# rounak-meyur/revs-admm

Measured on NVIDIA B200. Metric: home_hours_scheduled_per_sec, higher is better.
Workload: dtype f64

## Files before the change

include/revs_admm.h:

```cpp
#ifndef REVS_ADMM_H
#define REVS_ADMM_H

#include <stdint.h>

#ifdef __cplusplus
extern "C" {
#endif

#define REVS_OK 0
#define REVS_ERR_ARG 1
#define REVS_ERR_CUDA 2
#define REVS_ERR_INFEASIBLE 3
#define REVS_ERR_NOCONV 4

#define REVS_REL_VOLTAGE 0
#define REVS_REL_FLOW 1
#define REVS_REL_DROP 2

typedef struct revs_solver revs_solver;

typedef struct revs_stats {
    int64_t kernel_launches;
    int64_t gemm_launches;
    int64_t gemm_full_launches;
// ... 3 lines not shown
    int32_t max_working_set;
    double primal_residual;
    double dual_residual;
    double qp_flops;
    float gemm_ms;
    float gemm_full_ms;
    float home_ms;
    float dual_ms;
    float qp_ms;
    float qp_big_ms;
    float total_ms;
    float qp_warp_ms;
    float qp_init_ms;
    int64_t qp_columns;
    int64_t qp_warp_rounds;
} revs_stats;

const char* revs_last_error(void);
int revs_version(void);
int revs_device_count(int* count);

int revs_create(revs_solver** out, int device, int n_feeders, const int64_t* feeder_off, int T);
int revs_destroy(revs_solver* s);

int revs_set_sensitivity(revs_solver* s, int feeder, const double* R_res);

int revs_set_feeder_tree(revs_solver* s, int feeder, int n_nodes, const int32_t* parent,
                         const double* r, const int32_t* res_node);

int revs_set_feeder_trees(revs_solver* s, const int64_t* node_off, const int32_t* parent,
// ... 61 lines not shown
```

revs-admm_b200/_cabi.py:

```python
import ctypes as C
import os

import numpy as np

HERE = os.path.dirname(os.path.abspath(__file__))
LIB_PATH = os.environ.get("REVS_LIB") or os.path.join(HERE, "librevs_admm.so")

REVS_REL_VOLTAGE, REVS_REL_FLOW, REVS_REL_DROP = 0, 1, 2


class RevsError(RuntimeError):
    def __init__(self, code, msg):
        super().__init__(f"revs_admm error {code}: {msg}")
        self.code = code


class Stats(C.Structure):
    _fields_ = [("kernel_launches", C.c_int64), ("gemm_launches", C.c_int64), ("gemm_full_launches", C.c_int64),
                ("qp_outer_iterations", C.c_int64), ("qp_newton_iterations", C.c_int64),
                ("admm_iterations", C.c_int32), ("max_working_set", C.c_int32),
                ("primal_residual", C.c_double), ("dual_residual", C.c_double), ("qp_flops", C.c_double),
                ("gemm_ms", C.c_float), ("gemm_full_ms", C.c_float), ("home_ms", C.c_float), ("dual_ms", C.c_float),
                ("qp_ms", C.c_float), ("qp_big_ms", C.c_float), ("total_ms", C.c_float),
                ("qp_warp_ms", C.c_float), ("qp_init_ms", C.c_float), ("qp_columns", C.c_int64),
                ("qp_warp_rounds", C.c_int64)]

    def as_dict(self):
        return {k: getattr(self, k) for k, _ in self._fields_}


_P = C.c_void_p
_D = C.POINTER(C.c_double)
SIGNATURES = {
    "revs_last_error": ([], C.c_char_p),
    "revs_version": ([], C.c_int),
    "revs_device_count": ([C.POINTER(C.c_int)], C.c_int),
    "revs_create": ([C.POINTER(_P), C.c_int, C.c_int, C.POINTER(C.c_int64), C.c_int], C.c_int),
    "revs_destroy": ([_P], C.c_int),
    "revs_set_sensitivity": ([_P, C.c_int, _D], C.c_int),
    "revs_set_feeder_tree": ([_P, C.c_int, C.c_int, C.POINTER(C.c_int32), _D, C.POINTER(C.c_int32)], C.c_int),
    "revs_set_feeder_trees": ([_P, C.POINTER(C.c_int64), C.POINTER(C.c_int32), _D, C.POINTER(C.c_int32)], C.c_int),
    "revs_set_homes": ([_P, _D, C.POINTER(C.c_uint8), _D, _D, _D, C.POINTER(C.c_int32),
                        C.POINTER(C.c_int32)], C.c_int),
# ... 320 lines not shown
```

revs-admm_b200/csrc/kernels.cuh:

```cuda
#pragma once
#include <vector>

#include "common.cuh"

namespace revs {

struct HomeParams {
    const double* load;
    const double* p_est;
    const double* p_sch;
    const int* iter;
    const double* gamma;
    const double* cost;
    const uint8_t* has_ev;
    const double* rating;
    const int* start;
    const int* end;
    const int* n_min;
    const int* n_max;
    double* p_sch_new;
    double* p_ev;
    double* dsum;
    int first;
    int* infeasible;
// ... 115 lines not shown
struct ClassGateParams {
    const int* order_count;
    unsigned long long cond[kQpClasses];
    int first_gated;
};
cudaError_t launch_class_gate(const ClassGateParams& P, cudaStream_t stream);
cudaError_t qp_warp_prepare();
cudaError_t screen_prepare();
cudaError_t screen_tc5_prepare();

cudaError_t launch_utility_qp(const QpParams& P, int grid, int cls, cudaStream_t stream);
int qp_warp_max_n();
cudaError_t launch_qp_init(const QpParams& P, int max_warp_n, cudaStream_t stream);
int qp_warp_ctas_per_sm();
int qp_warp_m_max_default();
cudaError_t launch_utility_qp_warp(const QpParams& P, int nj, int ctas_per_sm, cudaStream_t stream);
cudaError_t launch_utility_qp_fast(const QpParams& P, cudaStream_t stream);
cudaError_t launch_order_columns(const QpParams& P, int mode, int* order, int* order_count, cudaStream_t stream);

struct TreeParams {
    const int64_t* zoff;
    const int* perm;
    const int* iperm;
    const double* c;
    const double* d;
    const double* e;
    const int* nodeA;
    const double* wA;
    const int* permB;
    const int* cnt;
    int* left;
// ... 99 lines not shown
```

revs-admm_b200/csrc/revs_capi.cu:

```cuda
#include <chrono>
#include <cstdarg>
#include <cstdio>
#include <cstring>
#include <algorithm>
#include <cstdlib>
#include <cmath>
#include <mutex>
#include <string>
#include <vector>

#include "../../include/revs_admm.h"
#include "kernels.cuh"

using namespace revs;

namespace {

thread_local std::string g_err;

int fail(int code, const char* fmt, ...) {
    char buf[512];
    va_list ap;
    va_start(ap, fmt);
    vsnprintf(buf, sizeof buf, fmt, ap);
// ... 128 lines not shown
    double *d_nt_rho = nullptr, *d_nt_ws = nullptr;
    double4* d_nt_ws4 = nullptr;
    double2* d_nt_ws2 = nullptr;
    int64_t nt_ws_stride = 0;
    int n_newton_cols = 0;
    size_t nt_sig = 0;
    double* d_gather = nullptr;
    int64_t gather_cap = 0;
    double* peer_gather[kGatherMaxPeers] = {};
    int gather_world = 1, gather_rank = 0;
    unsigned long long gather_seq = 0;
    GatherDev* d_gather_dev = nullptr;
    unsigned* d_gather_ticket = nullptr;
    int* d_gather_timeout = nullptr;
    bool use_warp_kernel = true;
    bool overlap_home = true;
    bool screen = true;
    int screen_impl = 0;
    void *d_maps_a = nullptr, *d_map_b = nullptr;
    int* d_bcol0 = nullptr;
    bool tc5_ready = false;
    int *d_pool_parent = nullptr, *d_pool_res = nullptr;
    double* d_pool_cumr = nullptr;
    int64_t* d_pool_off = nullptr;
    size_t pool_nodes = 0;
    size_t Rpool_elems = 0;
    bool rn2_valid = false;
    double *d_load = nullptr, *d_pest = nullptr, *d_psch[2] = {nullptr, nullptr}, *d_gamma = nullptr,
           *d_pev = nullptr, *d_soc = nullptr;
    uint8_t* d_has_ev = nullptr;
// ... 688 lines not shown
        }
        sp = timed ? span_begin(s, cl == 1 ? 3 : 4, s->sQ[cl]) : nullptr;
        CU(launch_utility_qp(Q, grid ? grid[cl] : s->ncols, cl, s->sQ[cl]));
        if (sp) span_end(sp, s->sQ[cl]);
        CU(cudaEventRecord(s->evQ[cl], s->sQ[cl]));
        s->stats.kernel_launches++;
    }
    if ((!use || use[0]) && s->use_warp_kernel && s->zg.warp_n > 0) {
        s->stats.qp_warp_rounds++;
        const int full = qp_warp_ctas_per_sm();
        if (s->zg.n_big > 0) {
            Q.list0 = kListBig;
            Q.nlists = kQpBuckets;
            Q.list_extra = -1;
            sp = timed ? span_begin(s, 7, s->sU) : nullptr;
            CU(launch_utility_qp_warp(Q, 10, full, s->sU));
            if (sp) span_end(sp, s->sU);
            s->stats.kernel_launches++;
        }
        if (s->zg.n_mid > 0) {
            Q.list0 = kQpClasses + kQpBuckets;
            Q.nlists = kQpBuckets;
            Q.list_extra = -1;
            sp = timed ? span_begin(s, 7, s->sU) : nullptr;
            CU(launch_utility_qp_warp(Q, s->zg.mid_max <= 192 ? 6 : 8, full, s->sU));
            if (sp) span_end(sp, s->sU);
            s->stats.kernel_launches++;
        }
        if (s->zg.n_small > 0) {
            sp = timed ? span_begin(s, 8, s->sU) : nullptr;
            if (s->use_fast) {
                CU(launch_utility_qp_fast(Q, s->sU));
                s->stats.kernel_launches++;
            }
            Q.list0 = kQpClasses;
            Q.nlists = s->use_fast ? 2 : kQpBuckets;
            Q.list_extra = s->use_fast ? kListLeftover : -1;
            CU(launch_utility_qp_warp(Q, 4, full, s->sU));
            Q.list_extra = -1;
            s->stats.kernel_launches++;
            if (sp) span_end(sp, s->sU);
        }
    }
    for (int cl = 1; cl < kQpClasses; ++cl)
        if (!use || use[cl]) CU(cudaStreamWaitEvent(s->sU, s->evQ[cl], 0));
    s->stats.gemm_launches++;
    s->stats.qp_outer_iterations++;
    return REVS_OK;
}

int check_device_flags(revs_solver* s) {
    if (s->h_cnt->infeasible)
        return fail(REVS_ERR_INFEASIBLE, "a home charging sub-problem is infeasible (SOC window vs plug-in window)");
// ... 1479 lines not shown
            CU(cudaStreamCreateWithPriority(&s->sQ[cl], cudaStreamNonBlocking, pr));
        }
        return REVS_OK;
    }
    if (!strcmp(name, "screen_impl")) {
        if (value != 0.0 && !s->tc5_ready) return fail(REVS_ERR_ARG, "tcgen05 screening kernel unavailable (T > 96 or tensor-map encoding failed)");
        s->screen_impl = value != 0.0 ? 1 : 0;
        return REVS_OK;
    }
    return fail(REVS_ERR_ARG, "unknown option '%s'", name);
}

int revs_get_stats(const revs_solver* s, revs_stats* out) {
    if (!s || !out) return fail(REVS_ERR_ARG, "bad arguments");
    *out = s->stats;
    return REVS_OK;
}

}
```

revs-admm_b200/csrc/utility_qp_warp.cu:

```cuda
#include <cstdlib>

#include <cuda_bf16.h>

#include "kernels.cuh"

namespace revs {

namespace {

#ifndef REVS_WARPS_PER_CTA
#define REVS_WARPS_PER_CTA 4
#endif
constexpr int kWarpsPerCta = REVS_WARPS_PER_CTA;
constexpr int kCtasPerSm = 16 / kWarpsPerCta;
constexpr int kHW = kWW + 1;
constexpr int kCacheDoubles = 1024;
constexpr double kArcMinW = 9.5367431640625e-07;
constexpr int kPdasMaxW = 40;
constexpr double kHessShiftW = 1e-12;
constexpr int kAddMaxW = 8;
constexpr int kPassMaxW = 10;
constexpr int kRecheckMaxW = 256;
constexpr int kHysteresisW = 8;

template <int CACHE>
struct WarpSmemT {
    double H[kWW * kHW];
    double L[kWW * kHW];
    double rows[CACHE];
};
#ifndef REVS_WARP_CTAS_SMALL
#define REVS_WARP_CTAS_SMALL (8 / REVS_WARPS_PER_CTA)
#endif
#ifndef REVS_WARP_CTAS_BIG
#define REVS_WARP_CTAS_BIG (8 / REVS_WARPS_PER_CTA)
#endif
#ifndef REVS_WARP_CACHE_BIG
#define REVS_WARP_CACHE_BIG 2560
#endif
template <int NJ> struct WarpCfg {
    static constexpr int kCache = NJ <= 4 ? kCacheDoubles : REVS_WARP_CACHE_BIG;
    static constexpr int kCtas = NJ <= 8 ? (NJ <= 4 ? kCtasPerSm : REVS_WARP_CTAS_SMALL) : REVS_WARP_CTAS_BIG;
};

struct WarpStats {
    unsigned long long its = 0;
    double flops = 0.0;
    int handed = 0, deferred = 0, max_ws = 0, cols = 0;
};

__device__ __forceinline__ double warp_bcast(double v, int src) { return __shfl_sync(0xffffffffu, v, src); }

template <int NJ>
__device__ __forceinline__ void recheck_rows(unsigned candk, const double* __restrict__ R, int ld, int n,
                                             const double (&gj)[NJ], double (&vub)[NJ]) {
    const int lane = threadIdx.x & 31;
    const unsigned full = 0xffffffffu;
    if (!__any_sync(full, candk != 0u)) return;
#pragma unroll 1
    for (int k = 0; k < NJ; ++k) {
        unsigned cand = __ballot_sync(full, (candk >> k) & 1u);
        while (cand) {
            int s[4], cnt = 0;
// ... 19 lines not shown
            double mine = 0.0;
            bool hit = false;
#pragma unroll
            for (int q = 0; q < 4; ++q)
                if (q < cnt && lane == s[q]) { mine = a[q]; hit = true; }
            if (hit) {
#pragma unroll
                for (int kk = 0; kk < NJ; ++kk)
                    if (kk == k) vub[kk] = mine;
            }
        }
    }
}

template <int NJ>
__device__ __forceinline__ void solve_column(const QpParams& P, const int4 ent, WarpSmemT<WarpCfg<NJ>::kCache>& sm, WarpStats& st) {
    constexpr int kCacheD = WarpCfg<NJ>::kCache;
    const int lane = threadIdx.x & 31;
    const unsigned full = 0xffffffffu;
    const int c = ent.x;
    const int n = ent.z & 0xffff, ld = ent.z >> 16;
    const int t = c % P.T;
    const size_t hoff = (size_t)ent.y;
    const double* __restrict__ R = P.Rpool + ((size_t)ent.w << 4);
    const size_t col = (size_t)t * P.Hp + hoff;
    const double* z = P.z_t + col;
    double* lam_g = P.lam_t + col;
    double* g = P.g_t + col;
    const double u = P.u, tol = P.tol;
    int* widx = P.widx + (size_t)c * kWMax;
    const int m_old = P.wcount[c];
    const bool solved_before = P.inner_ok[c] == 1;
    const int wi = lane < kWW ? widx[lane] : 0;

    long long tr_start = 0;
    if (P.trace) asm volatile("mov.u64 %0, %%globaltimer;" : "=l"(tr_start));
    const long long tr_clk0 = clock64();
    const double thr = (1.0 - kScreenMargin) * u;

    double zj[NJ], gj[NJ], g0[NJ], vub[NJ];
    unsigned inw = 0;
    unsigned candk = 0;
    if (P.v32_t) {
        const float* v32 = P.v32_t + col;
        float vf[NJ];
#pragma unroll
        for (int k = 0; k < NJ; ++k) {
            const int jc = min(lane + 32 * k, n - 1);
            zj[k] = z[jc];
            gj[k] = g[jc];
            vf[k] = v32[jc];
        }
        if (lane < (n + 15) / 16) asm volatile("prefetch.global.L2 [%0];" ::"l"(P.rmax + hoff + 16 * lane));
#pragma unroll
        for (int k = 0; k < NJ; ++k) {
            const bool in = lane + 32 * k < n;
            if (!in) { zj[k] = 0.0; gj[k] = 0.0; }
            g0[k] = gj[k];
            const double a = in ? (double)vf[k] : 0.0;
            vub[k] = kScreenUp * a;
            if (in && a > thr) candk |= 1u << k;
        }
    } else {
        const double* v64 = P.v_t + col;
#pragma unroll
        for (int k = 0; k < NJ; ++k) {
            const int jc = min(lane + 32 * k, n - 1);
            zj[k] = z[jc];
            gj[k] = g[jc];
            vub[k] = v64[jc];
        }
#pragma unroll
        for (int k = 0; k < NJ; ++k) {
            if (lane + 32 * k >= n) { zj[k] = 0.0; gj[k] = 0.0; vub[k] = 0.0; }
            g0[k] = gj[k];
        }
    }

    int idx = 0, m = 0;
    double lam = 0.0;
    if (m_old > 0) {
        const double l = lane < m_old ? lam_g[wi] : 0.0;
        const unsigned keep = __ballot_sync(full, lane < m_old && l > 0.0);
        m = __popc(keep);
        const int src = __fns(keep, 0, lane + 1);
        const int si = __shfl_sync(full, wi, src & 31);
        const double sl = __shfl_sync(full, l, src & 31);
        if (lane < m) { idx = si; lam = sl; }
#pragma unroll 1
        for (int a = 0; a < m; ++a) {
            const int h = __shfl_sync(full, idx, a);
            if ((h & 31) == lane) inw |= 1u << (h >> 5);
        }
        candk &= ~inw;
    }

    double flops = 0.0;
    int its_total = 0;
    bool changed = false;
    long long tph[4] = {0, 0, 0, 0}, tq0 = clock64(), tq1;
    int npass = 0;
#define WPHASE(i) do { if (P.trace) { tq1 = clock64(); tph[i] += tq1 - tq0; tq0 = tq1; } } while (0)
    auto trace_out = [&](int kind) {
        if (P.trace && lane == 0) {
            long long tr_end; unsigned smid;
            asm volatile("mov.u64 %0, %%globaltimer;" : "=l"(tr_end));
            asm volatile("mov.u32 %0, %%smid;" : "=r"(smid));
            long long* rec = P.trace + 12 * (size_t)c;
            rec[0] = tr_start; rec[1] = tr_end; rec[2] = smid; rec[3] = ((long long)m << 20) | its_total;
            for (int i = 0; i < 4; ++i) rec[4 + i] = tph[i];
            rec[8] = npass; rec[9] = kind; rec[10] = m_old; rec[11] = clock64() - tr_clk0;
        }
    };
    tph[0] = tq0 - tr_clk0;
    int exit_kind = 0, reason = 0;
    double grad = 0.0;

    for (int pass = 0;; ++pass) {
        recheck_rows<NJ>(candk, R, ld, n, gj, vub);
        candk = 0;
        WPHASE(pass == 0 ? 0 : 3);

        if (pass > 0) {
            const bool row = lane < m;
            unsigned drop = __ballot_sync(full, row && !(lam > 0.0));
            if (drop) {
                const unsigned keep = __ballot_sync(full, row && lam > 0.0);
                while (drop) {
                    const int a = __ffs(drop) - 1;
// ... 110 lines not shown
            if (l != l_in) changed = true;
            if (ok && l == l_in) its = 0;
            if (!ok) its = 0;
        }

        if (!ok) {
            const double scale = warp_sum(row ? P.rn2[hoff + idx] : 0.0) / (double)max(m, 1);
            const double shift = kHessShiftW * scale + 1e-300;
            double phi;
            {
                double acc = 0.0;
#pragma unroll
                for (int k = 0; k < NJ; ++k) acc = fma(gj[k], gj[k], acc);
                phi = 0.5 * warp_sum(acc) + u * warp_sum(row ? lam : 0.0);
            }
            double hrow[kWW];
#pragma unroll
            for (int q = 0; q < kWW; ++q) hrow[q] = 0.0;
            unsigned fbits = 0;
            bool have_H = false;

#pragma unroll 1
            for (; its < P.inner_max; ++its) {
                grad = 0.0;
#pragma unroll 1
                for (int a = 0; a < m; ++a) {
                    const double* rr = rowp(a);
                    double acc = 0.0;
#pragma unroll
                    for (int k = 0; k < NJ; ++k) {
                        const int j = lane + 32 * k;
                        if (j < n) acc = fma(rr[j], gj[k], acc);
                    }
// ... 25 lines not shown
                            for (int q = 0; q <= p; q += 2) {
                                const double* r0 = rowp(q);
                                const double* r1 = rowp(min(q + 1, p));
                                double a0 = 0.0, a1 = 0.0;
#pragma unroll
                                for (int k = 0; k < NJ; ++k) {
                                    const int j = lane + 32 * k;
                                    if (j < n) { a0 = fma(rp[k], r0[j], a0); a1 = fma(rp[k], r1[j], a1); }
                                }
#pragma unroll
                                for (int o = 16; o > 0; o >>= 1) {
                                    a0 += __shfl_xor_sync(full, a0, o);
                                    a1 += __shfl_xor_sync(full, a1, o);
                                }
                                if (lane == p) {
#pragma unroll
                                    for (int qq = 0; qq < kWW; ++qq) {
                                        if (qq == q) hrow[qq] = a0;
                                        if (qq == q + 1 && q + 1 <= p) hrow[qq] = a1;
                                    }
                                }
                            }
                        }
                        nupd = __reduce_add_sync(full, __popc(nowmask));
                    } else {
#pragma unroll 1
                        for (int k = 0; k < NJ; ++k) {
                            const bool now = (nowmask >> k) & 1u;
                            const bool was = (fbits >> k) & 1u;
                            unsigned chg = __ballot_sync(full, now != was);
                            const unsigned nowb = __ballot_sync(full, now);
                            while (chg) {
                                const int src = __ffs(chg) - 1;
                                chg &= chg - 1;
                                const int j = src + 32 * k;
                                const double sgn = ((nowb >> src) & 1u) ? 1.0 : -1.0;
                                const double ra = row ? (lane < ncache ? sm.rows[lane * ld + j] : R[(size_t)idx * ld + j]) : 0.0;
#pragma unroll
                                for (int q = 0; q < kWW; ++q) {
                                    const double rq = warp_bcast(ra, q);
                                    if (q <= lane) hrow[q] = fma(sgn * ra, rq, hrow[q]);
                                }
                                ++nupd;
                            }
                        }
                    }
                    fbits = nowmask;
                    have_H = true;
                    flops += (double)m * (m + 1) * nupd;
                    __syncwarp();
#pragma unroll
                    for (int q = 0; q < kWW; ++q)
                        if (row && q <= lane) { sm.H[lane * kHW + q] = hrow[q]; sm.H[q * kHW + lane] = hrow[q]; }
                    __syncwarp();
                }

                double b = 0.0;
#pragma unroll 1
                for (int q = 0; q < m; ++q) {
                    const double lq = warp_bcast(lam, q);
                    if (row && lq != 0.0) b = fma(sm.H[lane * kHW + q], lq, b);
                }
                b += shift * lam - grad;
                bool inA = row && (lam > 0.0 || grad < 0.0);
                double x = 0.0;
                bool pdas_ok = false;
#pragma unroll 1
                for (int guess = 0; guess < kPdasMaxW; ++guess) {
// ... 52 lines not shown
                    mu -= b;
                    const bool bad = row && (inA ? (x <= 0.0) : (mu < 0.0));
                    if (!__any_sync(full, bad)) { pdas_ok = true; break; }
                    if (bad) inA = !inA;
                }
                if (!pdas_ok) { bail = true; reason = 3; break; }

                const double dir = x - lam;
                double gt[NJ];
                double alpha = 1.0, phin = phi, lt = lam;
                bool stepped = false;
#pragma unroll 1
                for (; alpha >= kArcMinW; alpha *= 0.5) {
                    lt = row ? fmax(fma(alpha, dir, lam), 0.0) : 0.0;
                    {
                        double pi[NJ];
#pragma unroll
                        for (int k = 0; k < NJ; ++k) pi[k] = 0.0;
#pragma unroll 1
                        for (int a = 0; a < m; ++a) {
                            const double la = warp_bcast(lt, a);
                            const double* rr = rowp(a);
                            if (la != 0.0) {
#pragma unroll
                                for (int k = 0; k < NJ; ++k) {
                                    const int j = lane + 32 * k;
                                    if (j < n) pi[k] = fma(rr[j], la, pi[k]);
                                }
                            }
                        }
                        double acc = 0.0;
#pragma unroll
                        for (int k = 0; k < NJ; ++k) {
                            const int j = lane + 32 * k;
                            gt[k] = j < n ? fmax(zj[k] - pi[k], 0.0) : 0.0;
                            acc = fma(gt[k], gt[k], acc);
                        }
                        phin = 0.5 * warp_sum(acc) + u * warp_sum(row ? lt : 0.0);
                    }
                    flops += 2.0 * m * n;
                    const double slope = warp_sum(row ? grad * (lt - lam) : 0.0);
                    if (phin <= phi + 1e-4 * slope + 1e-14 * fabs(phi)) { stepped = true; break; }
                }
                if (!stepped) { bail = true; reason = 4; break; }
                lam = lt;
                phi = phin;
                changed = true;
#pragma unroll
                for (int k = 0; k < NJ; ++k) gj[k] = gt[k];
            }
        }
        its_total += its;
        WPHASE(2);
        if (bail || !ok) { exit_kind = 2; if (!reason) reason = 5; break; }

        double dp = 0.0;
#pragma unroll
        for (int k = 0; k < NJ; ++k) dp += fmax(gj[k] - g0[k], 0.0);
        dp = warp_sum(dp) * (1.0 + 1e-9);
        int ncand = 0;
        {
            const double* rmax = P.rmax + hoff;
            double rm[NJ];
#pragma unroll
            for (int k = 0; k < NJ; ++k) rm[k] = rmax[min(lane + 32 * k, n - 1)];
#pragma unroll
            for (int k = 0; k < NJ; ++k) {
                const int j = lane + 32 * k;
                if (j < n && !((inw >> k) & 1u)) {
                    const double bnd = dp > 0.0 ? fma(rm[k], dp, vub[k]) : vub[k];
                    if (bnd - u > tol) { candk |= 1u << k; ++ncand; }
                    else vub[k] = bnd;
                }
            }
            ncand = __reduce_add_sync(full, ncand);
        }
#pragma unroll
        for (int k = 0; k < NJ; ++k) g0[k] = gj[k];
        flops += 2.0 * n * min(ncand, kRecheckMaxW);
        if (ncand == 0) break;
        if (ncand > kRecheckMaxW) { exit_kind = 1; break; }
    }
    WPHASE(3);

    if (exit_kind == 2) {
        if (lane == 0) { P.cls[c] = 1; P.inner_ok[c] = 2; }
        ++st.handed;
        trace_out(2 + 16 * reason);
        return;
    }
    if (changed || m != m_old) {
        if (lane < m_old) lam_g[wi] = 0.0;
        __syncwarp();
        if (lane < m) { lam_g[idx] = lam; widx[lane] = idx; }
        if (changed) {
            __nv_bfloat16* gbf = P.gbf_t ? reinterpret_cast<__nv_bfloat16*>(P.gbf_t) + col : nullptr;
#pragma unroll
            for (int k = 0; k < NJ; ++k) {
                const int j = lane + 32 * k;
                if (j < n) {
                    g[j] = gj[k];
                    if (gbf) gbf[j] = __float2bfloat16_rn((float)gj[k]);
                }
            }
        }
    }
    if (lane == 0) {
        P.wcount[c] = m;
        P.inner_ok[c] = 1;
        if (exit_kind == 0) P.status[c] = 1;
    }
    if (exit_kind == 1) ++st.deferred;
    trace_out(exit_kind);
    st.its += (unsigned long long)its_total;
    st.flops += flops;
    st.max_ws = max(st.max_ws, m);
#undef WPHASE
}

}

__global__ void __launch_bounds__(256) qp_init_kernel(QpParams P, int max_warp_n) {
    const int lane = threadIdx.x & 31;
    const int c = blockIdx.x * (blockDim.x >> 5) + (threadIdx.x >> 5);
    if (blockIdx.x == 0 && threadIdx.x == 0 && P.round_ctr) {
        *P.round_ctr = 0;
        if (P.use_cond) cudaGraphSetConditional((cudaGraphConditionalHandle)P.cond_round, 1u);
// ... 71 lines not shown
        P.status[c] = 0;
        P.inner_ok[c] = 0;
        if (P.cand) P.cand[c] = 0;
    }
}

cudaError_t launch_qp_init(const QpParams& P, int max_warp_n, cudaStream_t stream) {
    const int wpc = 8;
    qp_init_kernel<<<(P.ncols + wpc - 1) / wpc, 32 * wpc, 0, stream>>>(P, max_warp_n);
    return cudaGetLastError();
}

template <int NJ>
__global__ void __launch_bounds__(32 * kWarpsPerCta, WarpCfg<NJ>::kCtas) utility_qp_warp_kernel(QpParams P) {
    extern __shared__ __align__(16) unsigned char smem_raw[];
    using Smem = WarpSmemT<WarpCfg<NJ>::kCache>;
    const int lane = threadIdx.x & 31, wib = threadIdx.x >> 5;
    Smem& sm = reinterpret_cast<Smem*>(smem_raw)[wib];
    const int l0 = P.list0, nl = P.nlists;
    int cnt[kQpBuckets], total = 0;
#pragma unroll
    for (int b = 0; b < kQpBuckets; ++b) {
        const int li = b < nl ? l0 + b : ((b == nl && P.list_extra >= 0) ? P.list_extra : -1);
        cnt[b] = li >= 0 ? P.order_count[li] : 0;
        total += cnt[b];
    }
    WarpStats st;
    for (;;) {
        int slot = 0;
        if (lane == 0) slot = atomicAdd(P.queue + l0, 1);
        slot = __shfl_sync(0xffffffffu, slot, 0);
        if (slot >= total) break;
        int b = 0;
#pragma unroll
        for (int bb = 0; bb < kQpBuckets - 1; ++bb)
            if (b == bb && slot >= cnt[bb]) { slot -= cnt[bb]; ++b; }
        const int li = b < nl ? l0 + b : P.list_extra;
        const int4 ent = P.order4[(size_t)(li - kQpClasses) * P.ncols + slot];
        solve_column<NJ>(P, ent, sm, st);
        ++st.cols;
        __syncwarp();
    }
    if (lane == 0) {
        if (st.its) atomicAdd(P.newton_its, st.its);
        if (st.flops > 0.0) atomicAdd(P.flops, (unsigned long long)st.flops);
        if (st.max_ws) atomicMax(P.max_ws, st.max_ws);
        if (st.cols) atomicAdd(P.cols, (unsigned long long)st.cols);
        if (st.handed) { atomicAdd(P.n_running, st.handed); atomicAdd(P.n_cls + 1, st.handed); }
        if (st.deferred) { atomicAdd(P.n_running, st.deferred); atomicAdd(P.n_cls + 0, st.deferred); }
    }
}

constexpr int kFastWarps = 8;

__global__ void __launch_bounds__(32 * kFastWarps, 4) utility_qp_fast_kernel(QpParams P) {
    constexpr int NJ = 4;
    const int lane = threadIdx.x & 31;
    const unsigned full = 0xffffffffu;
    const int l0 = kQpClasses + 2;
    const int c1 = P.order_count[l0], total = c1 + P.order_count[l0 + 1];
    const double u = P.u, tol = P.tol, thr = (1.0 - kScreenMargin) * u;
    unsigned long long its_sum = 0;
    double flops = 0.0;
    int cols = 0, passed = 0, maxws = 0;
    for (;;) {
// ... 187 lines not shown
    }
}

cudaError_t launch_utility_qp_fast(const QpParams& P, cudaStream_t stream) {
    int dev = 0, n_sm = 0;
    cudaError_t e = cudaGetDevice(&dev);
    if (e == cudaSuccess) e = cudaDeviceGetAttribute(&n_sm, cudaDevAttrMultiProcessorCount, dev);
    if (e != cudaSuccess) return e;
    utility_qp_fast_kernel<<<n_sm * 4, 32 * kFastWarps, 0, stream>>>(P);
    return cudaGetLastError();
}

int qp_warp_max_n() { return kWarpMaxN; }

static int g_warp_n_sm[4][64] = {};

template <int NJ>
static cudaError_t prepare_warp_nj(int* n_sm_out) {
    const int smem = (int)sizeof(WarpSmemT<WarpCfg<NJ>::kCache>) * kWarpsPerCta;
    int* n_sm = g_warp_n_sm[(NJ - 4) / 2];
    int dev = 0;
    cudaError_t e = cudaGetDevice(&dev);
    if (e != cudaSuccess) return e;
    dev &= 63;
    if (!n_sm[dev]) {
        int n = 0;
        e = cudaDeviceGetAttribute(&n, cudaDevAttrMultiProcessorCount, dev);
        if (e == cudaSuccess) e = cudaFuncSetAttribute(utility_qp_warp_kernel<NJ>, cudaFuncAttributeMaxDynamicSharedMemorySize, smem);
#ifndef REVS_WARP_NO_CARVEOUT
        if (e == cudaSuccess) e = cudaFuncSetAttribute(utility_qp_warp_kernel<NJ>, cudaFuncAttributePreferredSharedMemoryCarveout, cudaSharedmemCarveoutMaxShared);
#endif
        if (e != cudaSuccess) return e;
        n_sm[dev] = n;
    }
    if (n_sm_out) *n_sm_out = n_sm[dev];
    return cudaSuccess;
}

cudaError_t qp_warp_prepare() {
    cudaError_t e = prepare_warp_nj<4>(nullptr);
    if (e == cudaSuccess) e = prepare_warp_nj<6>(nullptr);
    if (e == cudaSuccess) e = prepare_warp_nj<8>(nullptr);
    if (e == cudaSuccess) e = prepare_warp_nj<10>(nullptr);
    return e;
}

template <int NJ>
static cudaError_t launch_warp_nj(const QpParams& P, int ctas_per_sm, cudaStream_t stream) {
    const int smem = (int)sizeof(WarpSmemT<WarpCfg<NJ>::kCache>) * kWarpsPerCta;
    int nsm = 0;
    cudaError_t e = prepare_warp_nj<NJ>(&nsm);
    if (e != cudaSuccess) return e;
    int n_sm[1] = {nsm};
    const int dev = 0;
    const int cmax = WarpCfg<NJ>::kCtas;
    ctas_per_sm = ctas_per_sm < 1 ? 1 : (ctas_per_sm > cmax ? cmax : ctas_per_sm);
    utility_qp_warp_kernel<NJ><<<n_sm[dev] * ctas_per_sm, 32 * kWarpsPerCta, smem, stream>>>(P);
    return cudaGetLastError();
}

cudaError_t launch_utility_qp_warp(const QpParams& P, int nj, int ctas_per_sm, cudaStream_t stream) {
    if (nj == 10) return launch_warp_nj<10>(P, ctas_per_sm, stream);
    if (nj == 8) return launch_warp_nj<8>(P, ctas_per_sm, stream);
    if (nj == 6) return launch_warp_nj<6>(P, ctas_per_sm, stream);
    return launch_warp_nj<4>(P, ctas_per_sm, stream);
}

int qp_warp_ctas_per_sm() { return kCtasPerSm; }
int qp_warp_m_max_default() { return kWW - kHysteresisW; }

}
```

revs-admm_b200/parallel.py:

```python
import os

import numpy as np


def shard_feeders(sizes, world_size, rank):
    sizes = np.asarray(sizes, dtype=np.int64)
    if world_size <= 1:
        return 0, len(sizes)
    cum = np.concatenate([[0], np.cumsum(sizes)])
    total = cum[-1]
    bounds = [int(np.searchsorted(cum, total * r / world_size, side="left")) for r in range(world_size + 1)]
    bounds[0], bounds[-1] = 0, len(sizes)
    for r in range(1, world_size + 1):
        bounds[r] = max(bounds[r], bounds[r - 1])
    return bounds[rank], bounds[rank + 1]


def allreduce_sums(sums, device=None):
    import torch
    import torch.distributed as dist
    if not (dist.is_available() and dist.is_initialized()) or dist.get_world_size() == 1:
        return np.asarray(sums, dtype=np.float64)
    t = torch.tensor(np.asarray(sums, dtype=np.float64), dtype=torch.float64, device=device or "cpu")
    dist.all_reduce(t, op=dist.ReduceOp.SUM)
# ... 237 lines not shown
        pe, gm = np.empty((self.H, self.T)), np.empty((self.H, self.T))

        def f(k):
            lo, hi = self.rows[k]
            pe[lo:hi], gm[lo:hi] = self.parts[k].estimate()
        self._each(f)
        return pe, gm

    def stats(self):
        sts = [p.stats() for p in self.parts]
        out = {}
        for key in sts[0]:
            vals = [s[key] for s in sts]
            if key in ("total_ms", "admm_iterations", "max_working_set"):
                out[key] = max(vals)
            elif key in ("primal_residual", "dual_residual"):
                w = [hi - lo for lo, hi in self.rows]
                out[key] = float(np.sqrt(sum(v * v * n for v, n in zip(vals, w)) / max(sum(w), 1)))
            else:
                out[key] = sum(vals)
        out["total_ms_sum"] = sum(s["total_ms"] for s in sts)
        out["pipelines"] = len(sts)
        return out
```

Before: 268.2 million.

## Raise warp QP kernel occupancy by moving per-lane arrays into shared memory

Moves the per-lane Hessian row accumulator (hrow) and the g0 gradient snapshot from registers into per-warp shared memory. The row cache is sized from the SM's shared-memory budget, and the CTAs per SM for the NJ=6/8/10 variants go from 8/warps to 12/warps. Per-warp stat counters become atomics issued at the point of use, and the granted occupancy is queried and clamped at launch. The aim is to cut register pressure so more warps can be resident. The cost is more shared-memory traffic in the Hessian update loop and a smaller row cache per warp.

After: 275.3 million, median of 6. 1.03x the previous value.

```diff
diff --git a/include/revs_admm.h b/include/revs_admm.h
--- a/include/revs_admm.h
+++ b/include/revs_admm.h
@@ -41,6 +41,7 @@
     float qp_init_ms;
     int64_t qp_columns;
     int64_t qp_warp_rounds;
+    int32_t qp_warp_ctas_per_sm[4];
 } revs_stats;
 
 const char* revs_last_error(void);
diff --git a/profiles/exp_r03_compare.py b/profiles/exp_r03_compare.py
--- /dev/null
+++ b/profiles/exp_r03_compare.py
@@ -0,0 +1,63 @@
+import glob
+import json
+import os
+import sys
+
+import numpy as np
+
+
+def load_line(path):
+    lines = [l for l in open(path).read().splitlines() if l.startswith("{")]
+    return json.loads(lines[-1]) if lines else None
+
+
+def same_dump(a, b):
+    names = sorted(os.path.basename(p) for p in glob.glob(os.path.join(a, "*.npy")))
+    if not names or names != sorted(os.path.basename(p) for p in glob.glob(os.path.join(b, "*.npy"))):
+        return {"equal": False, "why": "different or missing files"}
+    diff = [n for n in names if not np.array_equal(np.load(os.path.join(a, n)), np.load(os.path.join(b, n)))]
+    return {"equal": not diff, "arrays": len(names), "differ": diff}
+
+
+def main(out):
+    summary = {}
+    for b in ("base", "new"):
+        runs = [load_line(p) for p in sorted(glob.glob(os.path.join(out, f"bench_{b}_*.json")))]
+        runs = [r for r in runs if r]
+        if not runs:
+            continue
+        ms = [r["ms_per_step"] for r in runs]
+        dev = [r["device_ms_per_step"] for r in runs]
+        warp = [r["kernels"]["utility_qp"]["ms_warp_kernels"] for r in runs]
+        share = [r["share_of_device_time"]["utility_qp"] for r in runs]
+        summary[b] = {"runs": len(runs), "ms_per_step": ms, "ms_per_step_median": float(np.median(ms)),
+                      "ms_per_step_spread": float(max(ms) - min(ms)),
+                      "device_ms_per_step_median": float(np.median(dev)), "device_ms_per_step_spread": float(max(dev) - min(dev)),
+                      "ms_warp_kernels": warp, "ms_warp_kernels_median": float(np.median(warp)),
+                      "utility_qp_share": share}
+        cp = os.path.join(out, f"ctas_{b}.json")
+        if os.path.exists(cp):
+            summary[b]["qp_warp_ctas_per_sm"] = json.load(open(cp))
+    if "base" in summary and "new" in summary:
+        b, n = summary["base"], summary["new"]
+        noise = max(b["ms_per_step_spread"], n["ms_per_step_spread"])
+        gain = b["ms_per_step_median"] - n["ms_per_step_median"]
+        summary["step_gain_ms"] = gain
+        summary["step_gain_exceeds_spread"] = bool(gain > noise)
+        summary["warp_kernel_change"] = n["ms_warp_kernels_median"] / b["ms_warp_kernels_median"] - 1.0
+    dumps = {}
+    for a in sorted(glob.glob(os.path.join(out, "dump", "new_*"))):
+        i = a.rsplit("_", 1)[1]
+        for ref in sorted(glob.glob(os.path.join(out, "dump", "base_*"))):
+            dumps[f"new_{i} vs {os.path.basename(ref)}"] = same_dump(ref, a)
+    mf = os.path.join(out, "dump", "mf_base"), os.path.join(out, "dump", "mf_new")
+    if all(os.path.isdir(d) for d in mf):
+        dumps["multifeeder new vs base"] = same_dump(*mf)
+    summary["bit_identical"] = dumps
+    summary["all_bit_identical"] = bool(dumps) and all(v["equal"] for v in dumps.values())
+    json.dump(summary, open(os.path.join(out, "summary.json"), "w"), indent=1)
+    print(json.dumps(summary, indent=1))
+
+
+if __name__ == "__main__":
+    main(sys.argv[1])
diff --git a/profiles/exp_r03_ctas.py b/profiles/exp_r03_ctas.py
--- /dev/null
+++ b/profiles/exp_r03_ctas.py
@@ -0,0 +1,16 @@
+import json
+import os
+import sys
+
+sys.path.insert(0, os.path.dirname(os.path.dirname(os.path.abspath(__file__))))
+import bench
+import revs_admm_b200 as R
+
+wl = sys.argv[1] if len(sys.argv) > 1 else "synthetic-refshape-125k-homes-per-gpu-x96"
+trees, hm, cost, sizes, T = bench.make_rank_problem(wl, 0)
+with R.Solver(sizes, T, device=0) as s:
+    s.set_feeder_trees(trees)
+    s.set_homes(**hm)
+    s.set_tariff(cost)
+    s.solve_admm(**bench.ADMM)
+    print(json.dumps(s.stats()["qp_warp_ctas_per_sm"]))
diff --git a/revs-admm_b200/_cabi.py b/revs-admm_b200/_cabi.py
--- a/revs-admm_b200/_cabi.py
+++ b/revs-admm_b200/_cabi.py
@@ -23,10 +23,10 @@
                 ("gemm_ms", C.c_float), ("gemm_full_ms", C.c_float), ("home_ms", C.c_float), ("dual_ms", C.c_float),
                 ("qp_ms", C.c_float), ("qp_big_ms", C.c_float), ("total_ms", C.c_float),
                 ("qp_warp_ms", C.c_float), ("qp_init_ms", C.c_float), ("qp_columns", C.c_int64),
-                ("qp_warp_rounds", C.c_int64)]
+                ("qp_warp_rounds", C.c_int64), ("qp_warp_ctas_per_sm", C.c_int32 * 4)]
 
     def as_dict(self):
-        return {k: getattr(self, k) for k, _ in self._fields_}
+        return {k: list(v) if isinstance(v, C.Array) else v for k, v in ((k, getattr(self, k)) for k, _ in self._fields_)}
 
 
 _P = C.c_void_p
diff --git a/revs-admm_b200/csrc/kernels.cuh b/revs-admm_b200/csrc/kernels.cuh
--- a/revs-admm_b200/csrc/kernels.cuh
+++ b/revs-admm_b200/csrc/kernels.cuh
@@ -153,7 +153,7 @@
 cudaError_t launch_qp_init(const QpParams& P, int max_warp_n, cudaStream_t stream);
 int qp_warp_ctas_per_sm();
 int qp_warp_m_max_default();
-cudaError_t launch_utility_qp_warp(const QpParams& P, int nj, int ctas_per_sm, cudaStream_t stream);
+cudaError_t launch_utility_qp_warp(const QpParams& P, int nj, int ctas_per_sm, int* ctas_launched, cudaStream_t stream);
 cudaError_t launch_utility_qp_fast(const QpParams& P, cudaStream_t stream);
 cudaError_t launch_order_columns(const QpParams& P, int mode, int* order, int* order_count, cudaStream_t stream);
 
diff --git a/revs-admm_b200/csrc/revs_capi.cu b/revs-admm_b200/csrc/revs_capi.cu
--- a/revs-admm_b200/csrc/revs_capi.cu
+++ b/revs-admm_b200/csrc/revs_capi.cu
@@ -166,6 +166,7 @@
     unsigned* d_gather_ticket = nullptr;
     int* d_gather_timeout = nullptr;
     bool use_warp_kernel = true;
+    int warp_ctas[4] = {};
     bool overlap_home = true;
     bool screen = true;
     int screen_impl = 0;
@@ -884,7 +885,7 @@
             Q.nlists = kQpBuckets;
             Q.list_extra = -1;
             sp = timed ? span_begin(s, 7, s->sU) : nullptr;
-            CU(launch_utility_qp_warp(Q, 10, full, s->sU));
+            CU(launch_utility_qp_warp(Q, 10, full, &s->warp_ctas[3], s->sU));
             if (sp) span_end(sp, s->sU);
             s->stats.kernel_launches++;
         }
@@ -893,7 +894,8 @@
             Q.nlists = kQpBuckets;
             Q.list_extra = -1;
             sp = timed ? span_begin(s, 7, s->sU) : nullptr;
-            CU(launch_utility_qp_warp(Q, s->zg.mid_max <= 192 ? 6 : 8, full, s->sU));
+            const int nj = s->zg.mid_max <= 192 ? 6 : 8;
+            CU(launch_utility_qp_warp(Q, nj, full, &s->warp_ctas[(nj - 4) / 2], s->sU));
             if (sp) span_end(sp, s->sU);
             s->stats.kernel_launches++;
         }
@@ -906,7 +908,7 @@
             Q.list0 = kQpClasses;
             Q.nlists = s->use_fast ? 2 : kQpBuckets;
             Q.list_extra = s->use_fast ? kListLeftover : -1;
-            CU(launch_utility_qp_warp(Q, 4, full, s->sU));
+            CU(launch_utility_qp_warp(Q, 4, full, &s->warp_ctas[0], s->sU));
             Q.list_extra = -1;
             s->stats.kernel_launches++;
             if (sp) span_end(sp, s->sU);
@@ -2416,7 +2418,8 @@
 int revs_get_stats(const revs_solver* s, revs_stats* out) {
     if (!s || !out) return fail(REVS_ERR_ARG, "bad arguments");
     *out = s->stats;
-    return REVS_OK;
-}
-
-}
+    for (int i = 0; i < 4; ++i) out->qp_warp_ctas_per_sm[i] = s->warp_ctas[i];
+    return REVS_OK;
+}
+
+}
diff --git a/revs-admm_b200/csrc/utility_qp_warp.cu b/revs-admm_b200/csrc/utility_qp_warp.cu
--- a/revs-admm_b200/csrc/utility_qp_warp.cu
+++ b/revs-admm_b200/csrc/utility_qp_warp.cu
@@ -23,30 +23,40 @@
 constexpr int kRecheckMaxW = 256;
 constexpr int kHysteresisW = 8;
 
-template <int CACHE>
+#ifndef REVS_WARP_CTAS_SMALL
+#define REVS_WARP_CTAS_SMALL (12 / REVS_WARPS_PER_CTA)
+#endif
+#ifndef REVS_WARP_CTAS_BIG
+#define REVS_WARP_CTAS_BIG (12 / REVS_WARPS_PER_CTA)
+#endif
+constexpr int kSmemPerSm = 228 * 1024;
+constexpr int kSmemPerCtaReserved = 1024;
+
+template <int NJ> struct WarpCfg {
+    static constexpr int kCtas = NJ <= 8 ? (NJ <= 4 ? kCtasPerSm : REVS_WARP_CTAS_SMALL) : REVS_WARP_CTAS_BIG;
+    static constexpr int kFixedBytes = (2 * kWW * kHW + 32 * NJ) * (int)sizeof(double);
+    static constexpr int kCache = NJ <= 4 ? kCacheDoubles
+        : ((kSmemPerSm / kCtas - kSmemPerCtaReserved) / kWarpsPerCta - kFixedBytes) / (2 * (int)sizeof(double)) * 2;
+};
+
+template <int NJ>
 struct WarpSmemT {
     double H[kWW * kHW];
     double L[kWW * kHW];
-    double rows[CACHE];
+    double g0[32 * NJ];
+    double rows[WarpCfg<NJ>::kCache];
 };
-#ifndef REVS_WARP_CTAS_SMALL
-#define REVS_WARP_CTAS_SMALL (8 / REVS_WARPS_PER_CTA)
-#endif
-#ifndef REVS_WARP_CTAS_BIG
-#define REVS_WARP_CTAS_BIG (8 / REVS_WARPS_PER_CTA)
-#endif
-#ifndef REVS_WARP_CACHE_BIG
-#define REVS_WARP_CACHE_BIG 2560
-#endif
-template <int NJ> struct WarpCfg {
-    static constexpr int kCache = NJ <= 4 ? kCacheDoubles : REVS_WARP_CACHE_BIG;
-    static constexpr int kCtas = NJ <= 8 ? (NJ <= 4 ? kCtasPerSm : REVS_WARP_CTAS_SMALL) : REVS_WARP_CTAS_BIG;
-};
+template <int NJ> constexpr int kWarpSmemPerCta = (int)sizeof(WarpSmemT<NJ>) * kWarpsPerCta;
+static_assert(WarpCfg<6>::kCtas * (kWarpSmemPerCta<6> + kSmemPerCtaReserved) <= kSmemPerSm &&
+              WarpCfg<8>::kCtas * (kWarpSmemPerCta<8> + kSmemPerCtaReserved) <= kSmemPerSm &&
+              WarpCfg<10>::kCtas * (kWarpSmemPerCta<10> + kSmemPerCtaReserved) <= kSmemPerSm &&
+              WarpCfg<4>::kCtas * (kWarpSmemPerCta<4> + kSmemPerCtaReserved) <= kSmemPerSm,
+              "the warp QP kernels' CTAs per SM do not fit the shared memory of an SM");
 
 struct WarpStats {
     unsigned long long its = 0;
     double flops = 0.0;
-    int handed = 0, deferred = 0, max_ws = 0, cols = 0;
+    int max_ws = 0;
 };
 
 __device__ __forceinline__ double warp_bcast(double v, int src) { return __shfl_sync(0xffffffffu, v, src); }
@@ -96,7 +106,7 @@
 }
 
 template <int NJ>
-__device__ __forceinline__ void solve_column(const QpParams& P, const int4 ent, WarpSmemT<WarpCfg<NJ>::kCache>& sm, WarpStats& st) {
+__device__ __forceinline__ void solve_column(const QpParams& P, const int4 ent, WarpSmemT<NJ>& sm, WarpStats& st) {
     constexpr int kCacheD = WarpCfg<NJ>::kCache;
     const int lane = threadIdx.x & 31;
     const unsigned full = 0xffffffffu;
@@ -115,12 +125,16 @@
     const bool solved_before = P.inner_ok[c] == 1;
     const int wi = lane < kWW ? widx[lane] : 0;
 
-    long long tr_start = 0;
-    if (P.trace) asm volatile("mov.u64 %0, %%globaltimer;" : "=l"(tr_start));
-    const long long tr_clk0 = clock64();
+    long long* const trec = P.trace ? P.trace + 12 * (size_t)c : nullptr;
+    if (trec && lane == 0) {
+        long long t0;
+        asm volatile("mov.u64 %0, %%globaltimer;" : "=l"(t0));
+        trec[0] = t0;
+        trec[11] = clock64();
+    }
     const double thr = (1.0 - kScreenMargin) * u;
 
-    double zj[NJ], gj[NJ], g0[NJ], vub[NJ];
+    double zj[NJ], gj[NJ], vub[NJ];
     unsigned inw = 0;
     unsigned candk = 0;
     if (P.v32_t) {
@@ -138,7 +152,7 @@
         for (int k = 0; k < NJ; ++k) {
             const bool in = lane + 32 * k < n;
             if (!in) { zj[k] = 0.0; gj[k] = 0.0; }
-            g0[k] = gj[k];
+            sm.g0[32 * k + lane] = gj[k];
             const double a = in ? (double)vf[k] : 0.0;
             vub[k] = kScreenUp * a;
             if (in && a > thr) candk |= 1u << k;
@@ -155,7 +169,7 @@
 #pragma unroll
         for (int k = 0; k < NJ; ++k) {
             if (lane + 32 * k >= n) { zj[k] = 0.0; gj[k] = 0.0; vub[k] = 0.0; }
-            g0[k] = gj[k];
+            sm.g0[32 * k + lane] = gj[k];
         }
     }
 
@@ -180,21 +194,23 @@
     double flops = 0.0;
     int its_total = 0;
     bool changed = false;
-    long long tph[4] = {0, 0, 0, 0}, tq0 = clock64(), tq1;
     int npass = 0;
-#define WPHASE(i) do { if (P.trace) { tq1 = clock64(); tph[i] += tq1 - tq0; tq0 = tq1; } } while (0)
+#define WPHASE(i) do { if (trec && lane == 0) { const long long tq = clock64(); trec[4 + (i)] += tq - trec[1]; trec[1] = tq; } } while (0)
     auto trace_out = [&](int kind) {
-        if (P.trace && lane == 0) {
+        if (trec && lane == 0) {
             long long tr_end; unsigned smid;
             asm volatile("mov.u64 %0, %%globaltimer;" : "=l"(tr_end));
             asm volatile("mov.u32 %0, %%smid;" : "=r"(smid));
-            long long* rec = P.trace + 12 * (size_t)c;
-            rec[0] = tr_start; rec[1] = tr_end; rec[2] = smid; rec[3] = ((long long)m << 20) | its_total;
-            for (int i = 0; i < 4; ++i) rec[4 + i] = tph[i];
-            rec[8] = npass; rec[9] = kind; rec[10] = m_old; rec[11] = clock64() - tr_clk0;
+            trec[1] = tr_end; trec[2] = smid; trec[3] = ((long long)m << 20) | its_total;
+            trec[8] = npass; trec[9] = kind; trec[10] = m_old; trec[11] = clock64() - trec[11];
         }
     };
-    tph[0] = tq0 - tr_clk0;
+    if (trec && lane == 0) {
+        const long long tq = clock64();
+        trec[1] = tq;
+        trec[4] = tq - trec[11];
+        trec[5] = trec[6] = trec[7] = 0;
+    }
     int exit_kind = 0, reason = 0;
     double grad = 0.0;
 
@@ -335,9 +351,6 @@
                 for (int k = 0; k < NJ; ++k) acc = fma(gj[k], gj[k], acc);
                 phi = 0.5 * warp_sum(acc) + u * warp_sum(row ? lam : 0.0);
             }
-            double hrow[kWW];
-#pragma unroll
-            for (int q = 0; q < kWW; ++q) hrow[q] = 0.0;
             unsigned fbits = 0;
             bool have_H = false;
 
@@ -393,11 +406,8 @@
                                     a1 += __shfl_xor_sync(full, a1, o);
                                 }
                                 if (lane == p) {
-#pragma unroll
-                                    for (int qq = 0; qq < kWW; ++qq) {
-                                        if (qq == q) hrow[qq] = a0;
-                                        if (qq == q + 1 && q + 1 <= p) hrow[qq] = a1;
-                                    }
+                                    sm.H[p * kHW + q] = a0;
+                                    if (q + 1 <= p) sm.H[p * kHW + q + 1] = a1;
                                 }
                             }
                         }
@@ -415,10 +425,10 @@
                                 const int j = src + 32 * k;
                                 const double sgn = ((nowb >> src) & 1u) ? 1.0 : -1.0;
                                 const double ra = row ? (lane < ncache ? sm.rows[lane * ld + j] : R[(size_t)idx * ld + j]) : 0.0;
-#pragma unroll
-                                for (int q = 0; q < kWW; ++q) {
+#pragma unroll 4
+                                for (int q = 0; q < m; ++q) {
                                     const double rq = warp_bcast(ra, q);
-                                    if (q <= lane) hrow[q] = fma(sgn * ra, rq, hrow[q]);
+                                    if (row && q <= lane) sm.H[lane * kHW + q] = fma(sgn * ra, rq, sm.H[lane * kHW + q]);
                                 }
                                 ++nupd;
                             }
@@ -428,9 +438,9 @@
                     have_H = true;
                     flops += (double)m * (m + 1) * nupd;
                     __syncwarp();
-#pragma unroll
-                    for (int q = 0; q < kWW; ++q)
-                        if (row && q <= lane) { sm.H[lane * kHW + q] = hrow[q]; sm.H[q * kHW + lane] = hrow[q]; }
+#pragma unroll 1
+                    for (int q = 0; q < m; ++q)
+                        if (row && q < lane) sm.H[q * kHW + lane] = sm.H[lane * kHW + q];
                     __syncwarp();
                 }
 
@@ -513,9 +523,8 @@
                 for (; alpha >= kArcMinW; alpha *= 0.5) {
                     lt = row ? fmax(fma(alpha, dir, lam), 0.0) : 0.0;
                     {
-                        double pi[NJ];
-#pragma unroll
-                        for (int k = 0; k < NJ; ++k) pi[k] = 0.0;
+#pragma unroll
+                        for (int k = 0; k < NJ; ++k) gt[k] = 0.0;
 #pragma unroll 1
                         for (int a = 0; a < m; ++a) {
                             const double la = warp_bcast(lt, a);
@@ -524,7 +533,7 @@
 #pragma unroll
                                 for (int k = 0; k < NJ; ++k) {
                                     const int j = lane + 32 * k;
-                                    if (j < n) pi[k] = fma(rr[j], la, pi[k]);
+                                    if (j < n) gt[k] = fma(rr[j], la, gt[k]);
                                 }
                             }
                         }
@@ -532,7 +541,7 @@
 #pragma unroll
                         for (int k = 0; k < NJ; ++k) {
                             const int j = lane + 32 * k;
-                            gt[k] = j < n ? fmax(zj[k] - pi[k], 0.0) : 0.0;
+                            gt[k] = j < n ? fmax(zj[k] - gt[k], 0.0) : 0.0;
                             acc = fma(gt[k], gt[k], acc);
                         }
                         phin = 0.5 * warp_sum(acc) + u * warp_sum(row ? lt : 0.0);
@@ -555,7 +564,7 @@
 
         double dp = 0.0;
 #pragma unroll
-        for (int k = 0; k < NJ; ++k) dp += fmax(gj[k] - g0[k], 0.0);
+        for (int k = 0; k < NJ; ++k) dp += fmax(gj[k] - sm.g0[32 * k + lane], 0.0);
         dp = warp_sum(dp) * (1.0 + 1e-9);
         int ncand = 0;
         {
@@ -575,7 +584,7 @@
             ncand = __reduce_add_sync(full, ncand);
         }
 #pragma unroll
-        for (int k = 0; k < NJ; ++k) g0[k] = gj[k];
+        for (int k = 0; k < NJ; ++k) sm.g0[32 * k + lane] = gj[k];
         flops += 2.0 * n * min(ncand, kRecheckMaxW);
         if (ncand == 0) break;
         if (ncand > kRecheckMaxW) { exit_kind = 1; break; }
@@ -583,8 +592,7 @@
     WPHASE(3);
 
     if (exit_kind == 2) {
-        if (lane == 0) { P.cls[c] = 1; P.inner_ok[c] = 2; }
-        ++st.handed;
+        if (lane == 0) { P.cls[c] = 1; P.inner_ok[c] = 2; atomicAdd(P.n_running, 1); atomicAdd(P.n_cls + 1, 1); }
         trace_out(2 + 16 * reason);
         return;
     }
@@ -609,7 +617,7 @@
         P.inner_ok[c] = 1;
         if (exit_kind == 0) P.status[c] = 1;
     }
-    if (exit_kind == 1) ++st.deferred;
+    if (exit_kind == 1 && lane == 0) { atomicAdd(P.n_running, 1); atomicAdd(P.n_cls + 0, 1); }
     trace_out(exit_kind);
     st.its += (unsigned long long)its_total;
     st.flops += flops;
@@ -711,7 +719,7 @@
 template <int NJ>
 __global__ void __launch_bounds__(32 * kWarpsPerCta, WarpCfg<NJ>::kCtas) utility_qp_warp_kernel(QpParams P) {
     extern __shared__ __align__(16) unsigned char smem_raw[];
-    using Smem = WarpSmemT<WarpCfg<NJ>::kCache>;
+    using Smem = WarpSmemT<NJ>;
     const int lane = threadIdx.x & 31, wib = threadIdx.x >> 5;
     Smem& sm = reinterpret_cast<Smem*>(smem_raw)[wib];
     const int l0 = P.list0, nl = P.nlists;
@@ -735,17 +743,14 @@
         const int li = b < nl ? l0 + b : P.list_extra;
         const int4 ent = P.order4[(size_t)(li - kQpClasses) * P.ncols + slot];
         solve_column<NJ>(P, ent, sm, st);
-        ++st.cols;
         __syncwarp();
     }
     if (lane == 0) {
         if (st.its) atomicAdd(P.newton_its, st.its);
         if (st.flops > 0.0) atomicAdd(P.flops, (unsigned long long)st.flops);
         if (st.max_ws) atomicMax(P.max_ws, st.max_ws);
-        if (st.cols) atomicAdd(P.cols, (unsigned long long)st.cols);
-        if (st.handed) { atomicAdd(P.n_running, st.handed); atomicAdd(P.n_cls + 1, st.handed); }
-        if (st.deferred) { atomicAdd(P.n_running, st.deferred); atomicAdd(P.n_cls + 0, st.deferred); }
-    }
+    }
+    if (blockIdx.x == 0 && threadIdx.x == 0 && total) atomicAdd(P.cols, (unsigned long long)total);
 }
 
 constexpr int kFastWarps = 8;
@@ -963,56 +968,60 @@
 int qp_warp_max_n() { return kWarpMaxN; }
 
 static int g_warp_n_sm[4][64] = {};
+static int g_warp_granted[4][64] = {};
 
 template <int NJ>
-static cudaError_t prepare_warp_nj(int* n_sm_out) {
-    const int smem = (int)sizeof(WarpSmemT<WarpCfg<NJ>::kCache>) * kWarpsPerCta;
+static cudaError_t prepare_warp_nj(int* n_sm_out, int* granted_out) {
+    const int smem = kWarpSmemPerCta<NJ>;
     int* n_sm = g_warp_n_sm[(NJ - 4) / 2];
+    int* granted = g_warp_granted[(NJ - 4) / 2];
     int dev = 0;
     cudaError_t e = cudaGetDevice(&dev);
     if (e != cudaSuccess) return e;
     dev &= 63;
     if (!n_sm[dev]) {
-        int n = 0;
+        int n = 0, g = 0;
         e = cudaDeviceGetAttribute(&n, cudaDevAttrMultiProcessorCount, dev);
         if (e == cudaSuccess) e = cudaFuncSetAttribute(utility_qp_warp_kernel<NJ>, cudaFuncAttributeMaxDynamicSharedMemorySize, smem);
 #ifndef REVS_WARP_NO_CARVEOUT
         if (e == cudaSuccess) e = cudaFuncSetAttribute(utility_qp_warp_kernel<NJ>, cudaFuncAttributePreferredSharedMemoryCarveout, cudaSharedmemCarveoutMaxShared);
 #endif
+        if (e == cudaSuccess) e = cudaOccupancyMaxActiveBlocksPerMultiprocessor(&g, utility_qp_warp_kernel<NJ>, 32 * kWarpsPerCta, smem);
+        if (e == cudaSuccess && g < 1) e = cudaErrorLaunchOutOfResources;
         if (e != cudaSuccess) return e;
+        granted[dev] = g;
         n_sm[dev] = n;
     }
     if (n_sm_out) *n_sm_out = n_sm[dev];
+    if (granted_out) *granted_out = granted[dev];
     return cudaSuccess;
 }
 
 cudaError_t qp_warp_prepare() {
-    cudaError_t e = prepare_warp_nj<4>(nullptr);
-    if (e == cudaSuccess) e = prepare_warp_nj<6>(nullptr);
-    if (e == cudaSuccess) e = prepare_warp_nj<8>(nullptr);
-    if (e == cudaSuccess) e = prepare_warp_nj<10>(nullptr);
+    cudaError_t e = prepare_warp_nj<4>(nullptr, nullptr);
+    if (e == cudaSuccess) e = prepare_warp_nj<6>(nullptr, nullptr);
+    if (e == cudaSuccess) e = prepare_warp_nj<8>(nullptr, nullptr);
+    if (e == cudaSuccess) e = prepare_warp_nj<10>(nullptr, nullptr);
     return e;
 }
 
 template <int NJ>
-static cudaError_t launch_warp_nj(const QpParams& P, int ctas_per_sm, cudaStream_t stream) {
-    const int smem = (int)sizeof(WarpSmemT<WarpCfg<NJ>::kCache>) * kWarpsPerCta;
-    int nsm = 0;
-    cudaError_t e = prepare_warp_nj<NJ>(&nsm);
+static cudaError_t launch_warp_nj(const QpParams& P, int ctas_per_sm, int* ctas_launched, cudaStream_t stream) {
+    int n_sm = 0, granted = 0;
+    cudaError_t e = prepare_warp_nj<NJ>(&n_sm, &granted);
     if (e != cudaSuccess) return e;
-    int n_sm[1] = {nsm};
-    const int dev = 0;
-    const int cmax = WarpCfg<NJ>::kCtas;
+    const int cmax = min(WarpCfg<NJ>::kCtas, granted);
     ctas_per_sm = ctas_per_sm < 1 ? 1 : (ctas_per_sm > cmax ? cmax : ctas_per_sm);
-    utility_qp_warp_kernel<NJ><<<n_sm[dev] * ctas_per_sm, 32 * kWarpsPerCta, smem, stream>>>(P);
+    if (ctas_launched) *ctas_launched = ctas_per_sm;
+    utility_qp_warp_kernel<NJ><<<n_sm * ctas_per_sm, 32 * kWarpsPerCta, kWarpSmemPerCta<NJ>, stream>>>(P);
     return cudaGetLastError();
 }
 
-cudaError_t launch_utility_qp_warp(const QpParams& P, int nj, int ctas_per_sm, cudaStream_t stream) {
-    if (nj == 10) return launch_warp_nj<10>(P, ctas_per_sm, stream);
-    if (nj == 8) return launch_warp_nj<8>(P, ctas_per_sm, stream);
-    if (nj == 6) return launch_warp_nj<6>(P, ctas_per_sm, stream);
-    return launch_warp_nj<4>(P, ctas_per_sm, stream);
+cudaError_t launch_utility_qp_warp(const QpParams& P, int nj, int ctas_per_sm, int* ctas_launched, cudaStream_t stream) {
+    if (nj == 10) return launch_warp_nj<10>(P, ctas_per_sm, ctas_launched, stream);
+    if (nj == 8) return launch_warp_nj<8>(P, ctas_per_sm, ctas_launched, stream);
+    if (nj == 6) return launch_warp_nj<6>(P, ctas_per_sm, ctas_launched, stream);
+    return launch_warp_nj<4>(P, ctas_per_sm, ctas_launched, stream);
 }
 
 int qp_warp_ctas_per_sm() { return kCtasPerSm; }
diff --git a/revs-admm_b200/parallel.py b/revs-admm_b200/parallel.py
--- a/revs-admm_b200/parallel.py
+++ b/revs-admm_b200/parallel.py
@@ -275,6 +275,8 @@
             vals = [s[key] for s in sts]
             if key in ("total_ms", "admm_iterations", "max_working_set"):
                 out[key] = max(vals)
+            elif key == "qp_warp_ctas_per_sm":
+                out[key] = [max(v) for v in zip(*vals)]
             elif key in ("primal_residual", "dual_residual"):
                 w = [hi - lo for lo, hi in self.rows]
                 out[key] = float(np.sqrt(sum(v * v * n for v, n in zip(vals, w)) / max(sum(w), 1)))
```
